# amacati/gp-mpc

Hardware: AMD Instinct MI355X
Metric: GP-MPC control steps/sec, 2D quadrotor H=30 N=200, batch 1024 @1/2/4/8 GPU (higher is better)
Workload: dtype f64

## Files before the change

### gp-mpc_amd/csrc/gpmpc_common.h

```cpp
#pragma once
#include <hip/hip_runtime.h>
#include <cstdint>

namespace gpmpc {

constexpr int kMaxGP = 4;
constexpr int kMaxGPDim = 3;
constexpr int kMaxNX = 12;
constexpr int kMaxNU = 4;
constexpr int kMaxH = 63;
constexpr int kPhases = 12;
constexpr int kMaxParams = 16;
constexpr int kStatsSlots = 12;

enum ModelId : int32_t { kQuad2D = 0, kQuad3D = 1, kCartpole = 2 };

enum SolveStatus : int32_t { kSuccess = 0, kNaN = 1, kMaxIter = 2, kMinStep = 3, kQPFailure = 4 };

struct GPDev {
    const double* rows;
    const double* vrows;
    const double* linvT;
    const double* tX;
    const double* tW;
    int32_t ntile;
    double xbar[3];
    int32_t n;
    int32_t nv;
    int32_t d;
    const double* vroot;
    int32_t vroot_cols;
    int32_t vroot_rank;
    double inv_ell2;
    double sf2;
    double sn2;
};

struct ProblemDev {
    int32_t model;
    int32_t nx, nu, H;
    int32_t n_gp;
    int32_t use_gp;
    double dt;
    double cost_scale;
    double uh;
    double params[kMaxParams];
    double x_lo[kMaxNX], x_hi[kMaxNX], u_lo[kMaxNU], u_hi[kMaxNU];
    double q[kMaxNX], r[kMaxNU], u_eq[kMaxNU];
    const double* traj;
    int32_t traj_len;
    int32_t tighten;
    double icdf;
    double Acl[kMaxNX * kMaxNX];
    double K[kMaxNU * kMaxNX];
    const double* tgain;
    int32_t max_iter, qp_max_iter;
    double tol_stat, tol_eq, tol_ineq, tol_comp, qp_tol, qp_mu0;
    int32_t lin_gen;
    int32_t waves;
    int32_t n_cu;
    int32_t order_dispatch;
    int32_t seg;
    double seg_piv_rel;
    int32_t shift;
// ... 136 lines not shown
```

### gp-mpc_amd/csrc/sqp_kernel.hip

```cpp
#include <algorithm>
#include <type_traits>

#include "gpmpc_common.h"
#include "models.h"

#ifndef GPMPC_SEG_FALLBACK
#define GPMPC_SEG_FALLBACK 1
#endif
#ifndef GPMPC_SOLVE_STAMP
#define GPMPC_SOLVE_STAMP 1
#endif
#ifndef GPMPC_TIGHTEN_LDS
#define GPMPC_TIGHTEN_LDS 1
#endif
#ifndef GPMPC_LIN_EARLY
#define GPMPC_LIN_EARLY 1
#endif
#ifndef GPMPC_PHASE_LANE
#define GPMPC_PHASE_LANE 1
#endif

namespace gpmpc {

template <int NW>
__device__ __forceinline__ void wave_sync() {
    if constexpr (NW == 1) {
        __syncthreads();
    } else {
        __builtin_amdgcn_fence(__ATOMIC_RELEASE, "wavefront");
        asm volatile("s_waitcnt lgkmcnt(0)" ::: "memory");
        __builtin_amdgcn_fence(__ATOMIC_ACQUIRE, "wavefront");
        __builtin_amdgcn_wave_barrier();
    }
}
#define WSYNC() wave_sync<NWAVES>()

#ifdef GPMPC_TIMING
#define TPHASE(id)                                                   \
    do {                                                             \
        const unsigned long long t_ = __builtin_amdgcn_s_memtime();  \
        tacc[tcur] += t_ - tlast;                                    \
        tlast = t_;                                                  \
        tcur = (id);                                                 \
    } while (0)
#else
#define TPHASE(id) do { } while (0)
#endif

template <int CTRL>
__device__ __forceinline__ double dpp_d(double v) {
    const long long b = __double_as_longlong(v);
    const int lo = __builtin_amdgcn_update_dpp(0, (int)b, CTRL, 0xf, 0xf, false);
    const int hi = __builtin_amdgcn_update_dpp(0, (int)(b >> 32), CTRL, 0xf, 0xf, false);
    return __longlong_as_double(((long long)hi << 32) | (unsigned int)lo);
}
template <int CTRL, int BANK>
__device__ __forceinline__ double dpp_merge(double old, double v) {
    const long long o = __double_as_longlong(old), b = __double_as_longlong(v);
    const int lo = __builtin_amdgcn_update_dpp((int)o, (int)b, CTRL, 0xf, BANK, false);
    const int hi = __builtin_amdgcn_update_dpp((int)(o >> 32), (int)(b >> 32), CTRL, 0xf, BANK, false);
    return __longlong_as_double(((long long)hi << 32) | (unsigned int)lo);
}
__device__ __forceinline__ double xor16_d(double v) {
    const long long b = __double_as_longlong(v);
    const auto lo = __builtin_amdgcn_permlane16_swap((int)b, (int)b, false, false);
    const auto hi = __builtin_amdgcn_permlane16_swap((int)(b >> 32), (int)(b >> 32), false, false);
    const bool odd = threadIdx.x & 16;
    const unsigned int rl = odd ? lo[0] : lo[1], rh = odd ? hi[0] : hi[1];
    return __longlong_as_double(((long long)rh << 32) | rl);
}
__device__ __forceinline__ double xor32_d(double v) {
    const long long b = __double_as_longlong(v);
    const auto lo = __builtin_amdgcn_permlane32_swap((int)b, (int)b, false, false);
    const auto hi = __builtin_amdgcn_permlane32_swap((int)(b >> 32), (int)(b >> 32), false, false);
    const bool up = threadIdx.x & 32;
    const unsigned int rl = up ? lo[0] : lo[1], rh = up ? hi[0] : hi[1];
    return __longlong_as_double(((long long)rh << 32) | rl);
}
template <class Op>
__device__ __forceinline__ double wave_reduce(double v, Op op) {
    v = op(v, dpp_d<0x128>(v));
    v = op(v, dpp_d<0x124>(v));
    v = op(v, dpp_d<0x4E>(v));
    v = op(v, dpp_d<0xB1>(v));
    v = op(v, xor16_d(v));
    return op(v, xor32_d(v));
}
__device__ __forceinline__ double wave_max(double v) {
    return wave_reduce(v, [](double a, double b) { return fmax(a, b); });
}
__device__ __forceinline__ double wave_min(double v) {
    return wave_reduce(v, [](double a, double b) { return fmin(a, b); });
}
__device__ __forceinline__ double wave_sum(double v) {
    return wave_reduce(v, [](double a, double b) { return a + b; });
}

typedef double f64x4 __attribute__((ext_vector_type(4)));

// ... 91 lines not shown
    if (t < nt) finish(a0, w0);
#pragma unroll
    for (int e = 0; e < NE; ++e) out[(16 * e + lc) * 4 + lr] = acc[e];
}

template <int N, class F, int I = 0>
__device__ __forceinline__ void static_for(F&& f) {
    if constexpr (I < N) {
        f(std::integral_constant<int, I>{});
        static_for<N, F, I + 1>(static_cast<F&&>(f));
    }
}

template <int TS = 1>
__device__ __attribute__((noinline)) void gp_tiles_dispatch(const double* tX, const double* tW, int ntile,
                                                          const double* zb, const double* czz, double* out,
                                                          int lane, int ne, int t0 = 0) {
    switch (ne) {
        case 1: gp_tiles<1, TS>(tX, tW, ntile, zb, czz, out, lane, t0); break;
        case 2: gp_tiles<2, TS>(tX, tW, ntile, zb, czz, out, lane, t0); break;
        case 3:
            gp_tiles<2, TS>(tX, tW, ntile, zb, czz, out, lane, t0);
            gp_tiles<1, TS>(tX, tW, ntile, zb + 32 * 4, czz + 32, out + 32 * 4, lane, t0);
            break;
        default:
            gp_tiles<2, TS>(tX, tW, ntile, zb, czz, out, lane, t0);
            gp_tiles<2, TS>(tX, tW, ntile, zb + 32 * 4, czz + 32, out + 32 * 4, lane, t0);
            break;
    }
}

template <int ID>
constexpr int kDefaultWaves = (Model<ID>::NB + 1 > 16) ? 4 : 1;

template <int ID, int NW = kDefaultWaves<ID>, bool SEG = false>
struct SqpKernel {
    using M = Model<ID>;
    static constexpr int NX = M::NX, NU = M::NU, NB = M::NB, NGP = M::NGP, NUNC = M::NUNC;
    static constexpr int GS = NB + 1;
    static constexpr int kCostLin = (NB + 1 > 16) ? 5 : 3;
    static constexpr int PS = NX + 1;
    static constexpr int NBS = NB | 1;
    static constexpr int CB = 4;
    static constexpr int NCB = (NB + CB - 1) / CB;

    static constexpr bool kMfma = (NB + 1 <= 16) && (NX + 1 <= 8);
    static constexpr bool lds_mult = NW > 1 && kMfma;
    static constexpr int NWAVES = NW;
    static_assert(NW == 1 || NW == 4 || (NW == 2 && kMfma), "one wave per instance, two (single-tile models) or four: one per SIMD");
    static constexpr int PP = NX * (NX + 1) / 2 + NX;
    static constexpr int PO = NX * (NX + 1) / 2;
    static constexpr bool kSeg = SEG;
    static_assert(!SEG || (NW >= 2 && NB + 1 <= 16 && NX + 1 <= 8), "segment-parallel solve: single-tile models on >= 2 waves");
    static constexpr int LI = 8 + NU;
    static_assert(!SEG || LI + NX <= 16, "lambda slots in the 16-wide tile");
    static constexpr int KST = SEG ? 2 * NX + 1 : PS;
    static constexpr int PPB = SEG ? PP + NX * NX : PP;
    static constexpr int PXL = PP;
    static constexpr int NSEG = NW >= 4 ? 3 : 2;
    static constexpr int NBD = NSEG - 1;
    static constexpr int SB_V = 0, SB_LAM = SB_V + 256 * NBD, SB_XM = SB_LAM + 8 * NBD, SB_VL1 = SB_XM + 8 * NSEG,
                         SB_TI = SB_VL1 + 8 * NBD, SB_Y = SB_TI + NX * NX * NBD, SB_YV = SB_Y + NX * NX * NBD,
                         SB_PH = SB_YV + 8 * NBD, SB = SEG ? (SB_PH + PP * NBD + 7) / 8 * 8 : 0;

    struct Lds {
        double *G, *P, *K, *Rui, *hq, *gq, *dxv, *cd, *Acl, *dummy, *zero, *gz, *gc, *gs, *gsh;
        double* sb;
        double *Dq, *xs;
        double *lam, *pim;
        int* ctrl;
    };
    __host__ __device__ static size_t tight_scratch(int H) { return (size_t)H * NUNC; }
    __host__ __device__ static size_t gp_scratch(int H) {
        return (size_t)9 * NGP * 16 * ((H + 15) / 16) + (size_t)(NWAVES - 1) * 64 * ((H + 15) / 16);
    }
    __host__ __device__ static size_t p_region(int H) {
        const size_t pp = (size_t)(H + 1) * PPB;
        return pp > gp_scratch(H) ? pp : gp_scratch(H);
    }
    __host__ __device__ static size_t lds_doubles(int H) {
        const size_t common = (size_t)64
                              + (size_t)8
                              + (size_t)8
                              + (lds_mult ? (size_t)(H + 1) * 2 * NB + (size_t)H * NX : 0)
                              + (size_t)SB
                              + (size_t)H * NX * GS
                              + (size_t)H * NU * KST
                              + (size_t)H * NU * NU
                              + (size_t)(H + 1) * NBS * 2
                              + (size_t)(H + 1) * NX;
        if (kMfma) {
            const size_t acl = (size_t)H * NX * PS;
            return common + p_region(H) + (acl > tight_scratch(H) ? acl : tight_scratch(H))
                   + (NWAVES > 1 ? 64 : 0);
        }
        return common + p_region(H)
               + tight_scratch(H)
               + (NWAVES > 1 ? (size_t)(H + 1) * NB + 64 : 0);
    }
    __device__ static Lds carve(double* s, int H) {
        Lds L{};
        L.dummy = s; s += 64;
        L.zero = s;  s += 8;
        L.ctrl = reinterpret_cast<int*>(s);  s += 8;
        if constexpr (lds_mult) {
            L.lam = s; s += (size_t)(H + 1) * 2 * NB;
// ... 667 lines not shown
            *sk = kb;
            sk -= sk_st;
            *srui = rv;
            srui -= srui_st;
        };
        Stage s0, s1;
        load_stage(s0);
        int k = H - 1;
        for (; k >= 1; k -= 2) {
            load_stage(s1);
            stage(s0);
            if (k >= 2) load_stage(s0);
            stage(s1);
        }
        if (k == 0) stage(s0);
        return ok;
        }
    }

    template <bool full>
    __device__ static void acl_phase(const Lds& L, int H, int lane) {
        lane = phase_lane(lane);
        if constexpr (full) {
            for (int e = lane; e < H * NX; e += 64) {
                const int k = e / NX, i = e - k * NX;
                const double* G = L.G + (size_t)k * NX * GS + i * GS;
                const double* Kk = L.K + (size_t)k * NU * PS;
                double g[GS], kr[NU][PS];
#pragma unroll
                for (int j = 0; j < GS; ++j) g[j] = G[j];
#pragma unroll
                for (int a = 0; a < NU; ++a)
#pragma unroll
                    for (int j = 0; j < PS; ++j) kr[a][j] = Kk[a * PS + j];
                double* out = L.Acl + (size_t)k * NX * PS + i * PS;
#pragma unroll
                for (int j = 0; j < PS; ++j) {
                    double acc = (j < NX) ? g[j] : g[NB];
#pragma unroll
                    for (int a = 0; a < NU; ++a) acc = fma(g[NX + a], kr[a][j], acc);
                    out[j] = acc;
                }
            }
        } else {
            const int n = H * NX;
            for (int e0 = lane; e0 < n; e0 += 192) {
                double acc[3];
#pragma unroll
                for (int r = 0; r < 3; ++r) {
                    const int e = min(e0 + 64 * r, n - 1);
                    const int k = e / NX, i = e - k * NX;
                    const double* G = L.G + (size_t)k * NX * GS + i * GS;
                    const double* Kk = L.K + (size_t)k * NU * PS;
                    acc[r] = G[NB];
#pragma unroll
                    for (int a = 0; a < NU; ++a) acc[r] = fma(G[NX + a], Kk[a * PS + NX], acc[r]);
                }
#pragma unroll
                for (int r = 0; r < 3; ++r) {
                    const int e = e0 + 64 * r;
                    if (e < n) {
                        const int k = e / NX, i = e - k * NX;
                        L.Acl[(size_t)k * NX * PS + i * PS + NX] = acc[r];
                    }
                }
            }
        }
    }

    struct Mfma4Lane {
        int r, b, c, row, col;
    };
    __device__ static Mfma4Lane mfma4_lane(int lane) {
        Mfma4Lane q;
        q.r = lane >> 4;
        q.b = (lane >> 2) & 3;
        q.c = lane & 3;
        q.row = ((q.b >> 1) ? 4 : 0) + q.c;
        q.col = ((q.b == 1 || q.b == 2) ? 4 : 0) + q.r;
        return q;
    }
    template <class F>
    __device__ static double mfma4_vec(const Mfma4Lane& q, F&& vget) {
        const int idx = ((q.b == 1 || q.b == 2) ? 4 : 0) + q.r;
        return idx < NX ? vget(idx) : (idx == NX ? 1.0 : 0.0);
    }
    __device__ static double mfma4_stage(double a, double y, double& s) {
        const double d = __builtin_amdgcn_mfma_f64_4x4x4f64(a, y, 0.0, 0, 0, 0);
        s = d + dpp_d<0x12C>(d);
        return dpp_merge<0x12C, 0xA>(s, s);
    }

    __device__ static void mfma4_forward(const Lds& L, int H, int lane) {
        lane = phase_lane(lane);
        static_assert(NX >= 4 && NX + 1 <= 8, "homogeneous 8-vector");
        {
            const Mfma4Lane q = mfma4_lane(lane);
            const bool ld = q.row < NX && q.col <= NX;
            const double* src = ld ? L.Acl + q.row * PS + q.col : L.zero + ((q.row == NX && q.col == NX) ? 7 : 0);
            const int st = ld ? NX * PS : 0;
            const bool stlo = q.b == 0 && q.c == 0 && q.r < NX;
            const bool sthi = q.b == 2 && q.c == 0 && 4 + q.r < NX;
            double* out = stlo ? L.dxv + NX + q.r : (sthi ? L.dxv + NX + 4 + q.r : L.dummy);
            const int ost = (stlo || sthi) ? NX : 0;
            if (lane < NX) L.dxv[lane] = 0.0;
            double y = mfma4_vec(q, [](int) { return 0.0; });
            double an = *src;
            for (int k = 0; k < H; ++k) {
                const double a = an;
                src += (k + 1 < H) ? st : 0;
                an = *src;
                double s;
                y = mfma4_stage(a, y, s);
                *out = s;
                out += ost;
            }
        }
    }

    __device__ static void mfma4_vector_backward(const Lds& L, int H, int lane) {
        lane = phase_lane(lane);
        double* T = L.hq;
        double* VT = L.dxv;
        const int n = H * NX;
        struct TOps { double pr[NX], gc[NX]; };
        auto t_load = [&](int e, TOps& o) {
            const int k = e / NX, i = e - k * NX;
            const double* Pn = L.P + (size_t)(k + 1) * PP;
            const double* G = L.G + (size_t)k * NX * GS;
#pragma unroll
            for (int l = 0; l < NX; ++l) {
                o.pr[l] = Pn[i <= l ? pidx(i, l) : pidx(l, i)];
                o.gc[l] = G[l * GS + NB];
            }
        };
        auto t_dot = [](const TOps& o) {
            double acc = 0.0;
#pragma unroll
            for (int l = 0; l < NX; ++l) acc = fma(o.pr[l], o.gc[l], acc);
            return acc;
        };
        for (int e0 = lane; e0 < n; e0 += 128) {
            const int e1 = e0 + 64;
            const bool has1 = e1 < n;
            TOps o0, o1;
            t_load(e0, o0);
            t_load(has1 ? e1 : e0, o1);
            __builtin_amdgcn_sched_barrier(0);
            const double a0 = t_dot(o0), a1 = t_dot(o1);
            T[e0] = a0;
            if (has1) T[e1] = a1;
        }
        WSYNC();
        struct VOps { double g0, gu[NU], kc[NU], ac[NX], tk[NX]; };
        auto vt_load = [&](int e, VOps& o) {
            const int k = e / NX, i = e - k * NX;
            const double* A = L.Acl + (size_t)k * NX * PS;
            const double* Kk = L.K + (size_t)k * NU * PS;
            o.g0 = L.gq[k * NBS + i];
#pragma unroll
            for (int a = 0; a < NU; ++a) {
                o.kc[a] = Kk[a * PS + i];
                o.gu[a] = L.gq[k * NBS + NX + a];
            }
#pragma unroll
            for (int l = 0; l < NX; ++l) {
                o.ac[l] = A[l * PS + i];
                o.tk[l] = T[k * NX + l];
            }
        };
        auto vt_dot = [](const VOps& o) {
            double acc = o.g0;
#pragma unroll
            for (int a = 0; a < NU; ++a) acc = fma(o.kc[a], o.gu[a], acc);
#pragma unroll
            for (int l = 0; l < NX; ++l) acc = fma(o.ac[l], o.tk[l], acc);
            return acc;
        };
        for (int e0 = lane; e0 < n; e0 += 128) {
            const int e1 = e0 + 64;
            const bool has1 = e1 < n;
            VOps o0, o1;
            vt_load(e0, o0);
            vt_load(has1 ? e1 : e0, o1);
            __builtin_amdgcn_sched_barrier(0);
            const double a0 = vt_dot(o0), a1 = vt_dot(o1);
            VT[e0] = a0;
            if (has1) VT[e1] = a1;
        }
        WSYNC();
        {
            const Mfma4Lane q = mfma4_lane(lane);
            const bool lda = q.row < NX && q.col < NX, ldv = q.row < NX && q.col == NX;
            const double* src = lda ? L.Acl + (size_t)(H - 1) * NX * PS + q.col * PS + q.row
                                    : (ldv ? VT + (size_t)(H - 1) * NX + q.row
                                           : L.zero + ((q.row == NX && q.col == NX) ? 7 : 0));
            const int st = lda ? NX * PS : (ldv ? NX : 0);
            if (lane < NX) L.P[(size_t)H * PP + PO + lane] = L.gq[H * NBS + lane];
            double y = mfma4_vec(q, [&](int i) { return L.gq[H * NBS + i]; });
            const bool stlo = q.b == 0 && q.c == 0 && q.r < NX;
            const bool sthi = q.b == 2 && q.c == 0 && 4 + q.r < NX;
            double* out = stlo ? L.P + (size_t)(H - 1) * PP + PO + q.r
                               : (sthi ? L.P + (size_t)(H - 1) * PP + PO + 4 + q.r : L.dummy);
            const int ost = (stlo || sthi) ? PP : 0;
            double an = *src;
            for (int k = H - 1; k >= 0; --k) {
                const double a = an;
                src -= (k >= 1) ? st : 0;
                an = *src;
                double sv;
                y = mfma4_stage(a, y, sv);
                *out = sv;
                out -= ost;
            }
        }
        WSYNC();
        for (int e = lane; e < H * NU; e += 64) {
            const int k = e / NU, a = e - k * NU;
            const double* G = L.G + (size_t)k * NX * GS;
            const double* pn = L.P + (size_t)(k + 1) * PP + PO;
            double gb[NU][NX], tp[NX], gqv[NU], rui[NU];
#pragma unroll
            for (int b2 = 0; b2 < NU; ++b2) {
                gqv[b2] = L.gq[k * NBS + NX + b2];
                rui[b2] = L.Rui[(size_t)k * NU * NU + a * NU + b2];
#pragma unroll
                for (int l = 0; l < NX; ++l) gb[b2][l] = G[l * GS + NX + b2];
            }
#pragma unroll
            for (int l = 0; l < NX; ++l) tp[l] = T[k * NX + l] + pn[l];
            __builtin_amdgcn_sched_barrier(0);
            double kf = 0.0;
#pragma unroll
            for (int b2 = 0; b2 < NU; ++b2) {
                double acc = gqv[b2];
#pragma unroll
                for (int l = 0; l < NX; ++l) acc = fma(gb[b2][l], tp[l], acc);
                kf = fma(rui[b2], acc, kf);
            }
            L.K[(size_t)k * NU * PS + a * PS + NX] = -kf;
        }
        WSYNC();
    }

    __device__ static void recover_step_mfma(const Lds& L, int H, int lane, double (&dd)[NB], double (&dpi)[NX]) {
        lane = phase_lane(lane);
        const bool on = lane <= H;
        const int kk = min(lane, H - 1);
        double dx[NX], dxn[NX];
#pragma unroll
        for (int i = 0; i < NX; ++i) {
            dx[i] = (on && lane >= 1) ? L.dxv[(size_t)lane * NX + i] : 0.0;
            dxn[i] = L.dxv[(size_t)(kk + 1) * NX + i];
        }
#pragma unroll
        for (int i = 0; i < NX; ++i) dd[i] = dx[i];
#pragma unroll
        for (int a = 0; a < NU; ++a) {
            double kr[PS];
#pragma unroll
            for (int j = 0; j < PS; ++j) kr[j] = L.K[(size_t)kk * NU * PS + a * PS + j];
            double du = kr[NX];
#pragma unroll
            for (int j = 0; j < NX; ++j) du = fma(kr[j], dx[j], du);
            dd[NX + a] = (lane < H) ? du : 0.0;
        }
        const double* Pn = L.P + (size_t)(kk + 1) * PP;
        double pp[PP];
#pragma unroll
        for (int q = 0; q < PP; ++q) pp[q] = Pn[q];
#pragma unroll
        for (int i = 0; i < NX; ++i) {
            double acc = pp[NX * (NX + 1) / 2 + i];
#pragma unroll
            for (int j = 0; j < NX; ++j) acc = fma(pp[i <= j ? pidx(i, j) : pidx(j, i)], dxn[j], acc);
            dpi[i] = (lane < H) ? -acc : 0.0;
        }
    }

    __host__ __device__ static int seg_start(int w, int H) { return (w * H) / NSEG; }
    __device__ static int lam_of(int t) { return (t >= LI && t < LI + NX) ? t - LI : -1; }
    __device__ static int phase_lane(int lane) {
        if constexpr (GPMPC_PHASE_LANE == 2 || (GPMPC_PHASE_LANE == 1 && (NWAVES == 1 || !kMfma)))
            asm volatile("" : "+v"(lane));
        return lane;
    }
    __device__ static double* pxl_at(const Lds& L, int k) { return L.P + (size_t)k * PPB + PXL; }

    template <bool AUG>
    struct Fac {
        static constexpr int CI = NX, UI = 8, NR = AUG ? 4 : 2;
        static_assert(NX + 1 <= 8 && NU <= 2 && UI + NU <= 16, "homogeneous tile layout");
        struct Stage { double g[2], d[3]; };
        double pn[NR];
        const double* pg[2];
        int gst[2];
        const double* pd[3];
        int dst[3];
        double* sp[2];
        int sp_st[2];
        double* sk;
        int sk_st;
        double* srui;
        int srui_st;
        bool lamc, lam2, lam3;
        double pend_p[2], pend_k, pend_r;
        bool ok;
        int lr, lc, lane;

        __device__ static int gcol(int t) { return t < NX ? t : (t == CI ? NB : ((t >= UI && t < UI + NU) ? NX + t - UI : -1)); }
        __device__ static int svar(int t) { return t < NX ? t : ((t >= UI && t < UI + NU) ? NX + t - UI : -1); }

        __device__ void init(const Lds& L, int H, int ln, int k0, int k1) {
            (void)k0;
            lane = phase_lane(ln);
            lr = lane >> 4;
            lc = lane & 15;
            const int gc_lc = gcol(lc), sv_lc = svar(lc), lm_lc = AUG ? lam_of(lc) : -1;
#pragma unroll
            for (int r = 0; r < NR; ++r) {
                const int t = lr + 4 * r;
                double v = 0.0;
                if constexpr (AUG) {
                    v = ((t < NX && lm_lc == t) || (lam_of(t) >= 0 && lam_of(t) == lc)) ? 1.0 : 0.0;
                } else {
                    if (t < NX && lc < NX) v = (t == lc) ? L.hq[H * NBS + t] : 0.0;
                    else if (t < NX && lc == CI) v = L.gq[H * NBS + t];
                    else if (t == CI && lc < NX) v = L.gq[H * NBS + lc];
                }
// ... 837 lines not shown
    __device__ static void ctpi_q(const Lds& L, int H, int kq, int vb, const double (&pi)[NX], double (&out)[NV]) {
        double pim1[NX];
#pragma unroll
        for (int i = 0; i < NX; ++i) pim1[i] = dpp_d<0x138>(pi[i]);
        const double* G = L.G + (size_t)min(kq, H - 1) * NX * GS + vb;
#pragma unroll
        for (int j = 0; j < NV; ++j) {
            const int v = vb + j;
            double acc = 0.0;
#pragma unroll
            for (int l = 0; l < NX; ++l) acc = fma(G[l * GS + j], pi[l], acc);
            double pm = (j < NX) ? pim1[j < NX ? j : 0] : 0.0;
            if constexpr (SPL) {
                const double ph = (NV + j < NX) ? pim1[NV + j < NX ? NV + j : 0] : 0.0;
                pm = vb ? ph : pm;
            }
            if constexpr (WSPL) {
#pragma unroll
                for (int q = 1; q < NWAVES; ++q) {
                    const int vq = q * NV + j;
                    if (vb == q * NV) pm = (vq < NX) ? pim1[vq < NX ? vq : 0] : 0.0;
                }
            }
            out[j] = (v < NB) ? (((kq < H) ? -acc : 0.0) + ((v < NX && kq >= 1 && kq <= H) ? pm : 0.0)) : 0.0;
        }
    }

    template <bool SPL, int NV>
    __device__ static void dyn_residual_q(const Lds& L, int H, int kq, const double (&d)[NV], const double (&c)[NX],
                                          double (&r)[NX]) {
        const int lane = threadIdx.x & 63;
        double df[NB], xn[NX];
        const int h = lane >> 5;
        double dother[NV];
#pragma unroll
        for (int j = 0; j < NV; ++j) dother[j] = SPL ? xor32_d(d[j]) : d[j];
#pragma unroll
        for (int v = 0; v < NB; ++v) df[v] = (!SPL || v / NV == h) ? d[v % NV] : dother[v % NV];
#pragma unroll
        for (int i = 0; i < NX; ++i) xn[i] = dpp_d<0x130>((!SPL || i / NV == h) ? d[i % NV] : dother[i % NV]);
        const double* G = L.G + (size_t)min(kq, H - 1) * NX * GS;
#pragma unroll
        for (int i = 0; i < NX; ++i) {
            double gr[NB];
#pragma unroll
            for (int j = 0; j < NB; ++j) gr[j] = G[i * GS + j];
            double acc = xn[i] - c[i];
#pragma unroll
            for (int j = 0; j < NB; ++j) acc = fma(-gr[j], df[j], acc);
            r[i] = (kq < H) ? acc : 0.0;
        }
    }

    template <int NV>
    __device__ static void recover_q(const Lds& L, int H, int kq, int vb, double (&dd)[NV], double (&dp)[NX]) {
        double ddf[NB];
        if constexpr (kSeg) recover_step_seg(L, H, kq, ddf, dp);
        else if constexpr (kMfma) recover_step_mfma(L, H, kq, ddf, dp);
        else recover_step(L, H, kq, ddf, dp);
#pragma unroll
        for (int j = 0; j < NV; ++j) {
            const double lo = ddf[j < NB ? j : 0];
            if constexpr (WSPL) {
                double v = lo;
#pragma unroll
                for (int q = 1; q < NWAVES; ++q)
                    if (vb == q * NV) v = ddf[q * NV + j < NB ? q * NV + j : 0];
                dd[j] = v;
            } else {
                const double up = (NV + j < NB) ? ddf[NV + j < NB ? NV + j : 0] : 0.0;
                dd[j] = vb ? up : lo;
            }
        }
    }

    static constexpr bool WSPL = NWAVES > 1 && !kMfma;
    template <bool SPL>
    __host__ __device__ static constexpr int nv_of() { return WSPL ? (NB + NWAVES - 1) / NWAVES : (SPL ? (NB + 1) / 2 : NB); }
    struct Tm {
        unsigned long long acc[kPhases];
        unsigned long long last;
        int cur;
    };
    __device__ static void XSYNC() {
        if constexpr (WSPL) __syncthreads();
        else wave_sync<NWAVES>();
    }
    __device__ static void xred2(const Lds& L, int lane, int wv, int& par, double vmax, double vsum, double& omax,
                                 double& osum) {
        vmax = wave_max(vmax);
        vsum = wave_sum(vsum);
        if constexpr (WSPL) {
            double* sl = L.xs + par * 2 * NWAVES;
            if (lane == 0) {
                sl[wv] = vmax;
                sl[NWAVES + wv] = vsum;
            }
            __syncthreads();
            vmax = sl[0];
            vsum = sl[NWAVES];
#pragma unroll
            for (int q = 1; q < NWAVES; ++q) {
                vmax = fmax(vmax, sl[q]);
                vsum += sl[NWAVES + q];
            }
            par ^= 1;
        }
        omax = vmax;
        osum = vsum;
    }
    __device__ static double xmax(const Lds& L, int lane, int wv, int& par, double v) {
// ... 123 lines not shown
#pragma unroll
                for (int j = 0; j < NV; ++j) {
                    const bool av = avq(j);
                    const double rd = av ? fma(hd[j], d[j], gv[j]) - ll[j] + lu[j] + ctq[j] : 0.0;
                    const double rl = av ? d[j] - blo[j] - sl[j] : 0.0;
                    const double ru = av ? bup[j] - d[j] - su[j] : 0.0;
                    m_rd = fmax(m_rd, fabs(rd));
                    m_lu = fmax(m_lu, fmax(fabs(rl), fabs(ru)));
                    mu_l += av ? ll[j] * sl[j] + lu[j] * su[j] : 0.0;
                    if (on_q && vb + j < NB) {
                        const double hv = hd[j] + (av ? ll[j] * isl[j] + lu[j] * isu[j] : 0.0);
                        const double gqv = av ? rd + ll[j] + ll[j] * rl * isl[j] - lu[j] - lu[j] * ru * isu[j] : 0.0;
                        L.hq[k_q * NBS + vb + j] = hv;
                        L.gq[k_q * NBS + vb + j] = gqv;
                    }
                }
#pragma unroll
                for (int i = 0; i < NX; ++i) m_rb = fmax(m_rb, fabs(rp[i]));
                double mu, m_res;
                xred2(L, lane, wv, par, fmax(m_rd, fmax(m_rb, m_lu)), mu_l, m_res, mu);
                mu /= nc;
                if (!(mu == mu) || !(m_res == m_res)) { qp_ok = false; break; }
                if (m_res <= P.qp_tol && mu <= P.qp_tol) break;
                if (actu_q && !hi_half) {
#pragma unroll
                    for (int i = 0; i < NX; ++i)
                        if (!WSPL || xrow_of(i) == wv) L.G[(size_t)kq * NX * GS + i * GS + NB] = -rp[i];
                }
                XSYNC();
                TPHASE(4);
                double dd[NV], dp[NX];
                if constexpr (kSeg) {
                    const bool rok = seg_run(L, H, lane, kCmdSegFactor);
                    if (!rok) { qp_ok = false; break; }
                    TPHASE(9);
                    recover_q<NV>(L, H, kq, vb, dd, dp);
                    TPHASE(3);
                } else if constexpr (kMfma) {
                    bool rok = true;
                    if (wv == 0) {
                        rok = mfma_backward_h(L, H, lane);
                        WSYNC();
                        TPHASE(8);
                        if (rok) acl_phase<true>(L, H, lane);
                        WSYNC();
                        TPHASE(6);
                        if (rok) mfma4_forward(L, H, lane);
                        WSYNC();
                    }
                    if constexpr (WSPL) rok = xall(L, lane, wv, par, rok);
                    if (!rok) { qp_ok = false; break; }
                    TPHASE(9);
                    recover_q<NV>(L, H, kq, vb, dd, dp);
                    TPHASE(3);
                } else {
                    static_assert(kMfmaBig, "stage products must fit one (mfma_backward_h) or two (mfma_backward_big) tiles");
                    bool rok = true;
                    if (wv == 0) {
                        rok = mfma_backward_big(L, H, lane);
                        WSYNC();
                        TPHASE(6);
                        if (rok) valu_forward_big(L, H, lane);
                    }
                    if constexpr (WSPL) rok = xall(L, lane, wv, par, rok);
                    if (!rok) { qp_ok = false; break; }
                    TPHASE(3);
                    recover_q<NV>(L, H, kq, vb, dd, dp);
                }
                double rmax = 1.0, mua_l = 0.0;
#pragma unroll
                for (int j = 0; j < NV; ++j) {
                    if (avq(j)) {
                        const double rl = d[j] - blo[j] - sl[j];
                        const double ru = bup[j] - d[j] - su[j];
                        const double ql = (dd[j] + rl) * isl[j], qu = (-dd[j] + ru) * isu[j];
                        rmax = fmax(rmax, fmax(fmax(-ql, -qu), fmax(1.0 + ql, 1.0 + qu)));
                    }
                }
                const double a_aff = fast_rcp(xmax(L, lane, wv, par, rmax));
#pragma unroll
                for (int j = 0; j < NV; ++j) {
                    if (avq(j)) {
                        const double rl = d[j] - blo[j] - sl[j];
                        const double ru = bup[j] - d[j] - su[j];
                        const double dsl = dd[j] + rl, dsu = -dd[j] + ru;
                        const double ql = dsl * isl[j], qu = dsu * isu[j];
                        mua_l += ll[j] * fma(-a_aff, 1.0 + ql, 1.0) * fma(a_aff, dsl, sl[j]) +
                                 lu[j] * fma(-a_aff, 1.0 + qu, 1.0) * fma(a_aff, dsu, su[j]);
                    }
                }
                const double mu_aff = xsum(L, lane, wv, par, mua_l) / nc;
                const double sr = mu_aff / mu;
                const double smu = sr * sr * sr * mu;
                double dda[NV];
#pragma unroll
                for (int j = 0; j < NV; ++j) {
                    dda[j] = dd[j];
                    if (on_q && avq(j)) {
                        const double rl = d[j] - blo[j] - sl[j];
                        const double ru = bup[j] - d[j] - su[j];
                        const double dsl = dd[j] + rl, dsu = -dd[j] + ru;
                        const double dll = -ll[j] * fma(dsl, isl[j], 1.0);
                        const double dlu = -lu[j] * fma(dsu, isu[j], 1.0);
                        L.gq[k_q * NBS + vb + j] += (dll * dsl - smu) * isl[j] - (dlu * dsu - smu) * isu[j];
                    }
                }
                XSYNC();
                TPHASE(5);
                if constexpr (kSeg) {
                    (void)seg_run(L, H, lane, kCmdSegVector);
                    TPHASE(9);
                    recover_q<NV>(L, H, kq, vb, dd, dp);
                    TPHASE(3);
                } else if constexpr (kMfma) {
                    if (wv == 0) {
                        mfma4_vector_backward(L, H, lane);
                        TPHASE(8);
                        acl_phase<false>(L, H, lane);
                        WSYNC();
                        TPHASE(6);
                        mfma4_forward(L, H, lane);
                        WSYNC();
                    }
                    XSYNC();
                    TPHASE(9);
                    recover_q<NV>(L, H, kq, vb, dd, dp);
                    TPHASE(3);
                } else {
                    if (wv == 0) {
                        valu_vector_big(L, H, lane);
                        TPHASE(6);
                        valu_forward_big(L, H, lane);
                    }
                    XSYNC();
                    TPHASE(3);
                    recover_q<NV>(L, H, kq, vb, dd, dp);
                }
                rmax = 1.0;
                double dsl[NV], dsu[NV], dll[NV], dlu[NV];
#pragma unroll
                for (int j = 0; j < NV; ++j) {
                    dsl[j] = dsu[j] = dll[j] = dlu[j] = 0.0;
                    if (avq(j)) {
                        const double rl = d[j] - blo[j] - sl[j];
                        const double ru = bup[j] - d[j] - su[j];
                        const double dsla = dda[j] + rl, dsua = -dda[j] + ru;
                        const double dlla = -ll[j] * fma(dsla, isl[j], 1.0);
                        const double dlua = -lu[j] * fma(dsua, isu[j], 1.0);
                        const double rml = ll[j] * sl[j] + dlla * dsla - smu;
                        const double rmu = lu[j] * su[j] + dlua * dsua - smu;
                        dsl[j] = dd[j] + rl;
                        dsu[j] = -dd[j] + ru;
                        dll[j] = (-rml - ll[j] * dsl[j]) * isl[j];
                        dlu[j] = (-rmu - lu[j] * dsu[j]) * isu[j];
                        const double ill = fast_rcp(ll[j]), ilu = fast_rcp(lu[j]);
                        rmax = fmax(rmax, fmax(fmax(-dsl[j] * isl[j], -dsu[j] * isu[j]),
                                               fmax(-dll[j] * ill, -dlu[j] * ilu)));
                    }
                }
                const double alpha = fmin(1.0, 0.995 * fast_rcp(xmax(L, lane, wv, par, rmax)));
#pragma unroll
                for (int j = 0; j < NV; ++j) {
                    if (avq(j)) {
                        d[j] = fma(alpha, dd[j], d[j]);
                        sl[j] = fma(alpha, dsl[j], sl[j]);
                        su[j] = fma(alpha, dsu[j], su[j]);
                        ll[j] = fma(alpha, dll[j], ll[j]);
                        lu[j] = fma(alpha, dlu[j], lu[j]);
                    }
                }
                if (actu_q) {
#pragma unroll
                    for (int i = 0; i < NX; ++i) piq[i] = fma(alpha, dp[i], piq[i]);
                }
            }
        }
        qit_out = qit;
        return qp_ok;
    }

// ... 350 lines not shown
#pragma unroll
                for (int i = 0; i < NX; ++i) t[i] = pi_s[i];
#pragma unroll
                for (int i = 0; i < NX; ++i) pi_l[i] = t[i];
            }
        }
        if (S.tight != nullptr && on) {
#pragma unroll
            for (int v = 0; v < NB; ++v) S.tight[((size_t)b * (H + 1) + k) * NB + v] = tsd[v];
        }
        auto lbv = [&](int v) { return (v < NX ? P.x_lo[v] : P.u_lo[v - NX]) + tsd[v] - P.uh; };
        auto ubv = [&](int v) { return (v < NX ? P.x_hi[v] : P.u_hi[v - NX]) - tsd[v] + P.uh; };

        auto lin_store = [&](const double (&Fs)[NX]) {
            if (lin_b == nullptr) return;
            if (lane < H) {
#pragma unroll
                for (int i = 0; i < NX; ++i) L.G[(size_t)lane * NX * GS + i * GS + NB] = Fs[i];
            }
            WSYNC();
            for (int e = lane; e < H * NX * GS; e += 64) lin_b[e] = L.G[e];
        };
        int status = kMaxIter, it = 0, qp_total = 0;
        double res[4] = {0, 0, 0, 0};
        if (!x0_ok) status = kQPFailure;
        for (it = 0; x0_ok; ++it) {
            double lamL[NB], lamU[NB], pi[NX];
#pragma unroll
            for (int v = 0; v < NB; ++v) {
                const bool av = v < NX ? act_x : act_u;
                lamL[v] = av ? lam_l[v] : 0.0;
                lamU[v] = av ? lam_l[NB + v] : 0.0;
            }
#pragma unroll
            for (int i = 0; i < NX; ++i) pi[i] = act_u ? pi_l[i] : 0.0;
            double F[NX];
            TPHASE(1);
#ifdef GPMPC_TIMING
            unsigned long long* tgp = &tacc[11];
#else
            unsigned long long* tgp = nullptr;
#endif
            if (kLinEarly && it == 0 && lin_hit) {
#pragma unroll
                for (int i = 0; i < NX; ++i) F[i] = lin_F[i];
            } else if (it == 0 && lin_hit) {
                for (int e = lane; e < H * NX * GS; e += 64) L.G[e] = lin_b[e];
#pragma unroll
                for (int i = 0; i < NX; ++i) F[i] = (lane < H) ? lin_b[(size_t)lane * NX * GS + i * GS + NB] : 0.0;
            } else {
                linearize(P, L, H, lane, w, F, tgp);
            }
            WSYNC();
            TPHASE(2);
            double yr[NB];
#pragma unroll
            for (int i = 0; i < NX; ++i) yr[i] = P.traj[(size_t)tref * NX + i];
#pragma unroll
            for (int a = 0; a < NU; ++a) yr[NX + a] = P.u_eq[a];
            double ct[NB];
            ctpi(L, H, lane, pi, ct);
            double xn[NX];
#pragma unroll
            for (int i = 0; i < NX; ++i) xn[i] = dpp_d<0x130>(w[i]);
            double r_stat = 0.0, r_eq = 0.0, r_ineq = 0.0, r_comp = 0.0;
            double g[NB];
#pragma unroll
            for (int v = 0; v < NB; ++v) {
                const bool av = v < NX ? act_x : act_u;
                g[v] = av ? hdiag(P, v, lane, H) * (w[v] - yr[v]) : 0.0;
                if (av) {
                    const double lb = lbv(v), ub = ubv(v);
                    r_stat = fmax(r_stat, fabs(g[v] - lamL[v] + lamU[v] + ct[v]));
                    r_ineq = fmax(r_ineq, fmax(lb - w[v], w[v] - ub));
                    r_comp = fmax(r_comp, fmax(fabs(lamL[v] * (w[v] - lb)), fabs(lamU[v] * (ub - w[v]))));
                }
            }
            double cq[NX];
#pragma unroll
            for (int i = 0; i < NX; ++i) {
                cq[i] = act_u ? F[i] - xn[i] : 0.0;
                r_eq = fmax(r_eq, fabs(cq[i]));
            }
            if (lane == 0) {
#pragma unroll
                for (int i = 0; i < NX; ++i) {
                    r_ineq = fmax(r_ineq, fabs(x0[i] - w[i]));
                    r_ineq = fmax(r_ineq, fmax(P.x_lo[i] - P.uh - w[i], w[i] - P.x_hi[i] - P.uh));
                }
            }
            res[0] = wave_max(r_stat);
            res[1] = wave_max(r_eq);
            res[2] = wave_max(r_ineq);
            res[3] = wave_max(r_comp);
            if (!(res[0] == res[0] && res[1] == res[1] && res[2] == res[2] && res[3] == res[3])) { status = kNaN; break; }
            if (res[0] <= P.tol_stat && res[1] <= P.tol_eq && res[2] <= P.tol_ineq && res[3] <= P.tol_comp) {
                status = kSuccess;
                lin_store(F);
                break;
            }
            if (it == P.max_iter) { status = kMaxIter; lin_store(F); break; }

            auto qv = [&](const double (&full)[NB], int j) {
                const double lo = (j < NB) ? full[j < NB ? j : 0] : 0.0;
                if constexpr (!SPL) return lo;
                const double up = xor32_d((NV + j < NB) ? full[NV + j < NB ? NV + j : 0] : 0.0);
                return hi_half ? up : lo;
            };
            double blo[NV], bup[NV], gv[NV], hd[NV], d[NV], ll[NV], lu[NV], piq[NX], cqq[NX];
            if constexpr (WSPL) {
                if (on) {
#pragma unroll
                    for (int v = 0; v < NB; ++v) {
                        L.hq[(size_t)k * NBS + v] = lbv(v) - w[v];
                        L.gq[(size_t)k * NBS + v] = ubv(v) - w[v];
                        L.Dq[(size_t)k * NB + v] = g[v];
                    }
#pragma unroll
                    for (int i = 0; i < NX; ++i) L.dxv[(size_t)k * NX + i] = cq[i];
                }
                if (lane == 0) {
#pragma unroll
                    for (int i = 0; i < NX; ++i) L.xs[4 * NWAVES + i] = x0[i] - w[i];
                    L.ctrl[0] = -2;
                }
                __syncthreads();
                qp_setup_pub<NV>(P, L, H, lane, 0, blo, bup, gv, hd, d, cqq);
            } else {
                double lbm[NB], ubm[NB], hdf[NB], d0[NB];
#pragma unroll
                for (int v = 0; v < NB; ++v) {
                    lbm[v] = lbv(v) - w[v];
                    ubm[v] = ubv(v) - w[v];
                    hdf[v] = hdiag(P, v, lane, H);
                    d0[v] = (lane == 0 && v < NX) ? x0[v] - w[v] : 0.0;
                }
#pragma unroll
                for (int j = 0; j < NV; ++j) {
                    blo[j] = qv(lbm, j);
                    bup[j] = qv(ubm, j);
                    gv[j] = qv(g, j);
                    hd[j] = qv(hdf, j);
                    d[j] = qv(d0, j);
                }
#pragma unroll
                for (int i = 0; i < NX; ++i) {
                    if constexpr (SPL) {
                        const double o = xor32_d(cq[i]);
                        cqq[i] = hi_half ? o : cq[i];
                    } else {
                        cqq[i] = cq[i];
                    }
                }
            }
            int qit = 0;
            const bool qp_ok = qp_ipm<SPL, NV>(P, L, H, lane, 0, blo, bup, gv, hd, d, cqq, ll, lu, piq, qit, tm);
            if constexpr (WSPL) qp_publish_step<NV>(L, H, lane, 0, d);
            qp_total += qit;
            TPHASE(2);
            if (!qp_ok) { status = kQPFailure; break; }
            if (on_q) {
#pragma unroll
                for (int j = 0; j < NV; ++j) {
                    if (vb + j < NB) {
                        const bool ab = avq(j);
                        lam_q[vb + j] = ab ? ll[j] : 0.0;
                        lam_q[NB + vb + j] = ab ? lu[j] : 0.0;
                    }
                }
            }
            bool fin = true;
#pragma unroll
            for (int v = 0; v < NB; ++v) {
                double dv = (v < NV) ? d[v < NV ? v : 0] : 0.0;
                if constexpr (WSPL) dv = L.Dq[(size_t)k * NB + v];
                if constexpr (SPL) {
                    const double up = xor32_d(d[v >= NV ? v - NV : 0]);
                    dv = (v >= NV) ? up : dv;
                }
                const bool av = v < NX ? (act_x || lane == 0) : act_u;
                if (av) w[v] += dv;
                fin = fin && (w[v] == w[v]);
            }
            if (act_u) {
#pragma unroll
                for (int i = 0; i < NX; ++i) pi_l[i] = piq[i];
            }
            if (lane == 0) {
#pragma unroll
                for (int i = 0; i < NX; ++i) w[i] = x0[i];
            }
            if (wave_min(fin ? 1.0 : 0.0) < 0.5) { status = kNaN; break; }
        }
        TPHASE(7);
#ifdef GPMPC_TIMING
        if (lane == 0 && io.timing != nullptr)
            for (int q = 0; q < kPhases; ++q) io.timing[(size_t)b * kPhases + q] = tacc[q];
#endif
        double* xo = S.x + (size_t)b * (H + 1) * NX;
        double* uo = S.u + (size_t)b * H * NU;
        const bool good = (status == kSuccess) || (status == kMaxIter);
        if constexpr (kLM) WSYNC();
        if (good) {
            if (on) {
#pragma unroll
                for (int i = 0; i < NX; ++i) xo[k * NX + i] = w[i];
                if constexpr (kLM) {
#pragma unroll
                    for (int v = 0; v < 2 * NB; ++v) lam_g[v] = lam_l[v];
                }
            }
            if (act_u) {
// ... 348 lines not shown
```

Before: 3.076 million.

## Solve IPM corrector as delta system to skip backward T products

Adds a delta-form corrector for the single-wave MFMA path. The second (corrector) backward/recovery pass now solves only for the gradient increment, zeroing the affine residual term, and adds the predictor's dpi and step back in. This lets the vector backward pass skip the T = P*G products and the Acl*T dot terms. It also adds finer timing phase ids, which only take effect under the timing build. The risk is numerical drift from splitting the solve into a sum of two solves, and correctness depends on hq holding the predictor dpi when the recovery reads it.

New measurement: 3.118 million, median of 6. 1.4% higher.

```diff
diff --git a/gp-mpc_amd/csrc/gpmpc_common.h b/gp-mpc_amd/csrc/gpmpc_common.h
--- a/gp-mpc_amd/csrc/gpmpc_common.h
+++ b/gp-mpc_amd/csrc/gpmpc_common.h
@@ -9,7 +9,7 @@
 constexpr int kMaxNX = 12;
 constexpr int kMaxNU = 4;
 constexpr int kMaxH = 63;
-constexpr int kPhases = 12;
+constexpr int kPhases = 15;
 constexpr int kMaxParams = 16;
 constexpr int kStatsSlots = 12;
 
diff --git a/gp-mpc_amd/csrc/sqp_kernel.hip b/gp-mpc_amd/csrc/sqp_kernel.hip
--- a/gp-mpc_amd/csrc/sqp_kernel.hip
+++ b/gp-mpc_amd/csrc/sqp_kernel.hip
@@ -16,6 +16,9 @@
 #ifndef GPMPC_LIN_EARLY
 #define GPMPC_LIN_EARLY 1
 #endif
+#ifndef GPMPC_CORR_DELTA
+#define GPMPC_CORR_DELTA 1
+#endif
 #ifndef GPMPC_PHASE_LANE
 #define GPMPC_PHASE_LANE 1
 #endif
@@ -36,6 +39,11 @@
 #define WSYNC() wave_sync<NWAVES>()
 
 #ifdef GPMPC_TIMING
+#define TPHASE_LOADS(id)                                             \
+    do {                                                             \
+        asm volatile("s_waitcnt vmcnt(0) lgkmcnt(0)" ::: "memory"); \
+        TPHASE(id);                                                  \
+    } while (0)
 #define TPHASE(id)                                                   \
     do {                                                             \
         const unsigned long long t_ = __builtin_amdgcn_s_memtime();  \
@@ -45,6 +53,7 @@
     } while (0)
 #else
 #define TPHASE(id) do { } while (0)
+#define TPHASE_LOADS(id) do { } while (0)
 #endif
 
 template <int CTRL>
@@ -242,6 +251,7 @@
     static constexpr int PO = NX * (NX + 1) / 2;
     static constexpr bool kSeg = SEG;
     static_assert(!SEG || (NW >= 2 && NB + 1 <= 16 && NX + 1 <= 8), "segment-parallel solve: single-tile models on >= 2 waves");
+    static constexpr bool kCorrDelta = GPMPC_CORR_DELTA != 0 && kMfma && !SEG && NW == 1;
     static constexpr int LI = 8 + NU;
     static_assert(!SEG || LI + NX <= 16, "lambda slots in the 16-wide tile");
     static constexpr int KST = SEG ? 2 * NX + 1 : PS;
@@ -1015,9 +1025,15 @@
                     const int k = e / NX, i = e - k * NX;
                     const double* G = L.G + (size_t)k * NX * GS + i * GS;
                     const double* Kk = L.K + (size_t)k * NU * PS;
-                    acc[r] = G[NB];
-#pragma unroll
-                    for (int a = 0; a < NU; ++a) acc[r] = fma(G[NX + a], Kk[a * PS + NX], acc[r]);
+                    if constexpr (kCorrDelta) {
+                        acc[r] = G[NX] * Kk[NX];
+#pragma unroll
+                        for (int a = 1; a < NU; ++a) acc[r] = fma(G[NX + a], Kk[a * PS + NX], acc[r]);
+                    } else {
+                        acc[r] = G[NB];
+#pragma unroll
+                        for (int a = 0; a < NU; ++a) acc[r] = fma(G[NX + a], Kk[a * PS + NX], acc[r]);
+                    }
                 }
 #pragma unroll
                 for (int r = 0; r < 3; ++r) {
@@ -1083,11 +1099,11 @@
 
     __device__ static void mfma4_vector_backward(const Lds& L, int H, int lane) {
         lane = phase_lane(lane);
-        double* T = L.hq;
-        double* VT = L.dxv;
+        [[maybe_unused]] double* T = L.hq;
+        [[maybe_unused]] double* VT = L.dxv;
         const int n = H * NX;
         struct TOps { double pr[NX], gc[NX]; };
-        auto t_load = [&](int e, TOps& o) {
+        [[maybe_unused]] auto t_load = [&](int e, TOps& o) {
             const int k = e / NX, i = e - k * NX;
             const double* Pn = L.P + (size_t)(k + 1) * PP;
             const double* G = L.G + (size_t)k * NX * GS;
@@ -1097,28 +1113,30 @@
                 o.gc[l] = G[l * GS + NB];
             }
         };
-        auto t_dot = [](const TOps& o) {
+        [[maybe_unused]] auto t_dot = [](const TOps& o) {
             double acc = 0.0;
 #pragma unroll
             for (int l = 0; l < NX; ++l) acc = fma(o.pr[l], o.gc[l], acc);
             return acc;
         };
-        for (int e0 = lane; e0 < n; e0 += 128) {
-            const int e1 = e0 + 64;
-            const bool has1 = e1 < n;
-            TOps o0, o1;
-            t_load(e0, o0);
-            t_load(has1 ? e1 : e0, o1);
-            __builtin_amdgcn_sched_barrier(0);
-            const double a0 = t_dot(o0), a1 = t_dot(o1);
-            T[e0] = a0;
-            if (has1) T[e1] = a1;
-        }
-        WSYNC();
-        struct VOps { double g0, gu[NU], kc[NU], ac[NX], tk[NX]; };
+        if constexpr (!kCorrDelta) {
+            for (int e0 = lane; e0 < n; e0 += 128) {
+                const int e1 = e0 + 64;
+                const bool has1 = e1 < n;
+                TOps o0, o1;
+                t_load(e0, o0);
+                t_load(has1 ? e1 : e0, o1);
+                __builtin_amdgcn_sched_barrier(0);
+                const double a0 = t_dot(o0), a1 = t_dot(o1);
+                T[e0] = a0;
+                if (has1) T[e1] = a1;
+            }
+            WSYNC();
+        }
+        struct VOps { double g0, gu[NU], kc[NU], ac[kCorrDelta ? 1 : NX], tk[kCorrDelta ? 1 : NX]; };
         auto vt_load = [&](int e, VOps& o) {
             const int k = e / NX, i = e - k * NX;
-            const double* A = L.Acl + (size_t)k * NX * PS;
+            [[maybe_unused]] const double* A = L.Acl + (size_t)k * NX * PS;
             const double* Kk = L.K + (size_t)k * NU * PS;
             o.g0 = L.gq[k * NBS + i];
 #pragma unroll
@@ -1126,18 +1144,22 @@
                 o.kc[a] = Kk[a * PS + i];
                 o.gu[a] = L.gq[k * NBS + NX + a];
             }
-#pragma unroll
-            for (int l = 0; l < NX; ++l) {
-                o.ac[l] = A[l * PS + i];
-                o.tk[l] = T[k * NX + l];
+            if constexpr (!kCorrDelta) {
+#pragma unroll
+                for (int l = 0; l < NX; ++l) {
+                    o.ac[l] = A[l * PS + i];
+                    o.tk[l] = T[k * NX + l];
+                }
             }
         };
         auto vt_dot = [](const VOps& o) {
             double acc = o.g0;
 #pragma unroll
             for (int a = 0; a < NU; ++a) acc = fma(o.kc[a], o.gu[a], acc);
-#pragma unroll
-            for (int l = 0; l < NX; ++l) acc = fma(o.ac[l], o.tk[l], acc);
+            if constexpr (!kCorrDelta) {
+#pragma unroll
+                for (int l = 0; l < NX; ++l) acc = fma(o.ac[l], o.tk[l], acc);
+            }
             return acc;
         };
         for (int e0 = lane; e0 < n; e0 += 128) {
@@ -1191,7 +1213,7 @@
                 for (int l = 0; l < NX; ++l) gb[b2][l] = G[l * GS + NX + b2];
             }
 #pragma unroll
-            for (int l = 0; l < NX; ++l) tp[l] = T[k * NX + l] + pn[l];
+            for (int l = 0; l < NX; ++l) tp[l] = kCorrDelta ? pn[l] : T[k * NX + l] + pn[l];
             __builtin_amdgcn_sched_barrier(0);
             double kf = 0.0;
 #pragma unroll
@@ -1206,6 +1228,7 @@
         WSYNC();
     }
 
+    template <bool ADD = false>
     __device__ static void recover_step_mfma(const Lds& L, int H, int lane, double (&dd)[NB], double (&dpi)[NX]) {
         lane = phase_lane(lane);
         const bool on = lane <= H;
@@ -1232,12 +1255,18 @@
         double pp[PP];
 #pragma unroll
         for (int q = 0; q < PP; ++q) pp[q] = Pn[q];
+        [[maybe_unused]] double da[NX];
+        if constexpr (ADD) {
+#pragma unroll
+            for (int i = 0; i < NX; ++i) da[i] = L.hq[kk * NBS + i];
+        }
 #pragma unroll
         for (int i = 0; i < NX; ++i) {
             double acc = pp[NX * (NX + 1) / 2 + i];
 #pragma unroll
             for (int j = 0; j < NX; ++j) acc = fma(pp[i <= j ? pidx(i, j) : pidx(j, i)], dxn[j], acc);
-            dpi[i] = (lane < H) ? -acc : 0.0;
+            if constexpr (ADD) dpi[i] = (lane < H) ? da[i] - acc : 0.0;
+            else dpi[i] = (lane < H) ? -acc : 0.0;
         }
     }
 
@@ -2181,11 +2210,12 @@
         }
     }
 
-    template <int NV>
+    template <int NV, bool ADD = false>
     __device__ static void recover_q(const Lds& L, int H, int kq, int vb, double (&dd)[NV], double (&dp)[NX]) {
         double ddf[NB];
+        static_assert(!ADD || kCorrDelta, "the delta corrector's recovery");
         if constexpr (kSeg) recover_step_seg(L, H, kq, ddf, dp);
-        else if constexpr (kMfma) recover_step_mfma(L, H, kq, ddf, dp);
+        else if constexpr (kMfma) recover_step_mfma<ADD>(L, H, kq, ddf, dp);
         else recover_step(L, H, kq, ddf, dp);
 #pragma unroll
         for (int j = 0; j < NV; ++j) {
@@ -2415,6 +2445,12 @@
                     if (!rok) { qp_ok = false; break; }
                     TPHASE(9);
                     recover_q<NV>(L, H, kq, vb, dd, dp);
+                    if constexpr (kCorrDelta) {
+                        if (actu_q && !hi_half) {
+#pragma unroll
+                            for (int i = 0; i < NX; ++i) L.hq[kq * NBS + i] = dp[i];
+                        }
+                    }
                     TPHASE(3);
                 } else {
                     static_assert(kMfmaBig, "stage products must fit one (mfma_backward_h) or two (mfma_backward_big) tiles");
@@ -2459,13 +2495,18 @@
 #pragma unroll
                 for (int j = 0; j < NV; ++j) {
                     dda[j] = dd[j];
+                    double dg = 0.0;
                     if (on_q && avq(j)) {
                         const double rl = d[j] - blo[j] - sl[j];
                         const double ru = bup[j] - d[j] - su[j];
                         const double dsl = dd[j] + rl, dsu = -dd[j] + ru;
                         const double dll = -ll[j] * fma(dsl, isl[j], 1.0);
                         const double dlu = -lu[j] * fma(dsu, isu[j], 1.0);
-                        L.gq[k_q * NBS + vb + j] += (dll * dsl - smu) * isl[j] - (dlu * dsu - smu) * isu[j];
+                        dg = (dll * dsl - smu) * isl[j] - (dlu * dsu - smu) * isu[j];
+                        if constexpr (!kCorrDelta) L.gq[k_q * NBS + vb + j] += dg;
+                    }
+                    if constexpr (kCorrDelta) {
+                        if (on_q && vb + j < NB) L.gq[k_q * NBS + vb + j] = dg;
                     }
                 }
                 XSYNC();
@@ -2487,8 +2528,12 @@
                     }
                     XSYNC();
                     TPHASE(9);
-                    recover_q<NV>(L, H, kq, vb, dd, dp);
+                    recover_q<NV, kCorrDelta>(L, H, kq, vb, dd, dp);
                     TPHASE(3);
+                    if constexpr (kCorrDelta) {
+#pragma unroll
+                        for (int j = 0; j < NV; ++j) dd[j] = dda[j] + dd[j];
+                    }
                 } else {
                     if (wv == 0) {
                         valu_vector_big(L, H, lane);
@@ -2945,12 +2990,13 @@
                 linearize(P, L, H, lane, w, F, tgp);
             }
             WSYNC();
-            TPHASE(2);
+            TPHASE(12);
             double yr[NB];
 #pragma unroll
             for (int i = 0; i < NX; ++i) yr[i] = P.traj[(size_t)tref * NX + i];
 #pragma unroll
             for (int a = 0; a < NU; ++a) yr[NX + a] = P.u_eq[a];
+            TPHASE_LOADS(13);
             double ct[NB];
             ctpi(L, H, lane, pi, ct);
             double xn[NX];
@@ -2993,6 +3039,7 @@
                 break;
             }
             if (it == P.max_iter) { status = kMaxIter; lin_store(F); break; }
+            TPHASE(14);
 
             auto qv = [&](const double (&full)[NB], int j) {
                 const double lo = (j < NB) ? full[j < NB ? j : 0] : 0.0;
@@ -3050,7 +3097,7 @@
             const bool qp_ok = qp_ipm<SPL, NV>(P, L, H, lane, 0, blo, bup, gv, hd, d, cqq, ll, lu, piq, qit, tm);
             if constexpr (WSPL) qp_publish_step<NV>(L, H, lane, 0, d);
             qp_total += qit;
-            TPHASE(2);
+            TPHASE(12);
             if (!qp_ok) { status = kQPFailure; break; }
             if (on_q) {
 #pragma unroll
```
